# netneurolab/pypyls

Measured on AMD Instinct MI355X. Metric: resamples/sec (perm+boot), behavioral_pls X(500x200000)/Y(500x50) fp64, higher is better.
Workload: dtype f64

## Files before the change

### pypyls_amd/csrc/plsx_compact.hip

```cpp
#include "plsx_internal.h"

using namespace plsxi;

namespace plsxi {

template <int MT, int KT, bool TAIL = false>
int launch_xprod_cboot(plsx_ctx* ctx, int nres, int nks_c, SplitEpi se, hipStream_t st)
{
    se.nmu = compact_moment_rows(ctx) ? ctx->Tp : 0;
    const size_t lds = compact_lds_bytes(MT, KT, 3, nks_c, se.npairs);
    HIPCHK(set_lds(k_xprod_compact<MT, KT, 3, TAIL>, lds));
    const int ncolblk = ceil_div(ctx->Bpad, 128);
    KTimer tm(ctx, KC_XPROD, st);
    hipLaunchKernelGGL((k_xprod_compact<MT, KT, 3, TAIL>), dim3(round_up(ncolblk, 8) * round_up(nres, 8)), dim3(256),
                       lds, st, ptr<double>(ctx->Afrag_c), (size_t)nks_c * MT * 64, ptr<double>(ctx->Xc), ctx->Bpad, nks_c,
                       ptr<double>(ctx->R), ctx->Bpad, ctx->Tpp, ptr<int>(ctx->out_row_c), ptr<int>(ctx->mom_idx_c),
                       ptr<double>(ctx->momn_m), nres, ncolblk, se);
    LAUNCHCHK();
    return 0;
}

int launch_cboot(plsx_ctx* ctx, int nres, int nks_c, SplitEpi se, hipStream_t st)
{
    const int MTc = ceil_div(ctx->Tp, 16);
    const bool tail = ctx->Tp - (MTc - 1) * 16 <= 4 && MTc >= 2;
    switch (MTc) {
        case 1: return launch_xprod_cboot<1, 12>(ctx, nres, nks_c, se, st);
        case 2: return tail ? launch_xprod_cboot<2, 6, true>(ctx, nres, nks_c, se, st)
                            : launch_xprod_cboot<2, 6>(ctx, nres, nks_c, se, st);
        case 3: return tail ? launch_xprod_cboot<3, 4, true>(ctx, nres, nks_c, se, st)
                            : launch_xprod_cboot<3, 4>(ctx, nres, nks_c, se, st);
        case 4: return tail ? launch_xprod_cboot<4, PLSX_CKT, true>(ctx, nres, nks_c, se, st)
                            : launch_xprod_cboot<4, PLSX_CKT>(ctx, nres, nks_c, se, st);
#define PLSX_CB(M, K) case M: return tail ? launch_xprod_cboot<M, K, true>(ctx, nres, nks_c, se, st) \
                                          : launch_xprod_cboot<M, K>(ctx, nres, nks_c, se, st);
        PLSX_CB(5, 2) PLSX_CB(6, 2) PLSX_CB(7, 1) PLSX_CB(8, 1) PLSX_CB(9, 1) PLSX_CB(10, 1) PLSX_CB(11, 1) PLSX_CB(12, 1) PLSX_CB(13, 1)
#undef PLSX_CB
        default: return fail(ctx, PLSX_ERR_STATE, "compact bootstrap blocks: T' > 208");
    }
}
template <int MT, int KT, bool TAIL = false, int EPI = 5>
int launch_xprod_compact(plsx_ctx* ctx, int m, int nks_c, SplitEpi se, hipStream_t st)
{
    const int J = ctx->J;
    const size_t lds = compact_lds_bytes(MT, KT, EPI, nks_c, J);
    se.off_pre = 0;
    HIPCHK(set_lds(k_xprod_compact<MT, KT, EPI, TAIL>, lds));
    const int ncolblk = ceil_div(ctx->Bpad, 128);
    KTimer tm(ctx, KC_XPROD, st);
    hipLaunchKernelGGL((k_xprod_compact<MT, KT, EPI, TAIL>), dim3(round_up(ncolblk, 8) * round_up(m, 8)), dim3(256), lds, st,
                       ptr<double>(ctx->Afrag_c), (size_t)nks_c * MT * 64, ptr<double>(ctx->Xc), ctx->Bpad, nks_c,
                       ptr<double>(ctx->R), ctx->Bpad, (EPI == 8 ? 1 : 2) * ctx->Tpp, ptr<int>(ctx->out_row_c), ptr<int>(ctx->mom_idx_c),
                       ptr<double>(ctx->momn_m), m, ncolblk, se);
    LAUNCHCHK();
    return 0;
}

int launch_csplit(plsx_ctx* ctx, int m, int nks_c, SplitEpi se, hipStream_t st, bool raw)
// ... 28 lines not shown
```

### pypyls_amd/csrc/plsx_core.hip

```cpp
#include "plsx_internal.h"
#include "plsx_resample.h"
using namespace plsxi;

namespace plsxi {

const char* const kKernelClassNames[KC_COUNT] = {"k_xprod", "k_gram", "k_small", "k_urot", "k_nt_gemm",
                                                 "k_ucorr_partial", "k_simpls_dual", "k_build_A", "k_xprod_moments",
                                                 "k_sd_cv_score", "k_sd_coef", "k_coef_prod", "k_percentile", "k_contrast", "k_mb_rownorm",
                                                 "k_sd_cv_class"};

int plan_groups(plsx_ctx* c)
{
    const bool mb = c->method == PLSX_MULTIBLOCK;
    c->scaled = ((c->method == PLSX_BEHAVIORAL || mb) && !c->cov) ? 1 : 0;
    c->momrows = ((c->method == PLSX_BEHAVIORAL && (!c->cov || c->cv_mom)) || (mb && !c->cov)) ? 1 : 0;
    const int Jw = c->momrows ? c->J : 0;
    c->gps = 0;
    c->h_slice_row0.clear(); c->h_slice_rows.clear(); c->h_slice_cell0.clear(); c->h_slice_ncell.clear();
    auto fit = [&](int mt) {
        int b = 0;
        for (int n = 1; n <= 512; ++n) {
            int td = ceil_div(n * c->Tp, 16), tw = Jw ? ceil_div(n * Jw, 16) : 0;
            if (td + 2 * tw <= mt && tw * 16 <= 48) b = n; else break;
        }
// ... 1231 lines not shown
    ctx->timing = enable ? 1 : 0;
    for (auto& ev : ctx->events) { (void)hipEventDestroy(ev.e0); (void)hipEventDestroy(ev.e1); }
    ctx->events.clear();
    ctx->timed_units = 0;
    ctx->nt_flops = 0.0;
    ctx->quad_series = 0;
    return PLSX_OK;
} PLSX_CATCH(ctx)

int plsx_last_timing(const plsx_ctx* cctx, double* out, int cap)
try {
    plsx_ctx* ctx = const_cast<plsx_ctx*>(cctx);
    if (!ctx || !out || cap < 1) return PLSX_ERR_ARG;
    double ms = 0.0;
    int launches = 0;
    for (auto& ev : ctx->events) {
        if (ev.cls != KC_XPROD) continue;
        float t = 0.f;
        if (hipEventSynchronize(ev.e1) == hipSuccess && hipEventElapsedTime(&t, ev.e0, ev.e1) == hipSuccess)
            ms += t;
        ++launches;
    }
    double crows = 0.0;
    if (ctx->last_compact_n > 0) {
        std::vector<int> cnt(ctx->last_compact_n);
        if (hipMemcpy(cnt.data(), ptr<int>(ctx->rowtab_c) + (size_t)ctx->last_compact_n * ctx->last_compact_ktot,
                      cnt.size() * sizeof(int), hipMemcpyDeviceToHost) == hipSuccess) {
            for (int c : cnt) crows += 4.0 * ((std::max(c, 1) + 3) / 4);
            crows /= (double)cnt.size() * ctx->S;
        }
    }
    const bool cmp = ctx->last_compact_n > 0;
    const auto uvar = [&](int nks) { return (double)(nks > 0 && ctx->urot_tail_l ? nks + 100 : nks); };
    double vals[23] = {ms, (double)launches, (double)(cmp ? 1 : (ctx->sepmom_used ? ctx->npg_d : ctx->npg)),
                       (double)(cmp ? ceil_div(ctx->Tp, 16) : (ctx->sepmom_used ? ctx->MTd : ctx->MT)),
                       (double)ctx->Gcap * ctx->npg, (double)ctx->timed_units, (double)use_dual(ctx), crows,
                       ctx->nt_flops, (double)ctx->quad_series, (double)ctx->quad_MT, (double)ctx->quad_gpl,
                       (double)ctx->urot_waves_l, (double)ctx->urot_splits_l, (double)ctx->urot_rps_l,
                       uvar(ctx->urot_nks_first), (double)ctx->gram_chunks_l, uvar(ctx->urot_nks_last),
                       (double)ctx->gram_kind_l, (double)ctx->split_blocks_l, (double)ctx->split_reader_l,
                       (double)(cmp && ctx->last_moment_rows ? 1 : 0), (double)ctx->last_perm_projected};
    int n = std::min(cap, 23);
    for (int i = 0; i < n; ++i) out[i] = vals[i];
    return n;
} PLSX_CATCH(const_cast<plsx_ctx*>(cctx))

int plsx_kernel_timing(const plsx_ctx* cctx, int kernel_class, double* ms_out, int* launches_out)
try {
    plsx_ctx* ctx = const_cast<plsx_ctx*>(cctx);
    if (!ctx || kernel_class < 0 || kernel_class >= KC_COUNT) return PLSX_ERR_ARG;
    double ms = 0.0;
    int launches = 0;
    for (auto& ev : ctx->events) {
        if (ev.cls != kernel_class) continue;
        float t = 0.f;
        if (hipEventSynchronize(ev.e1) == hipSuccess && hipEventElapsedTime(&t, ev.e0, ev.e1) == hipSuccess)
            ms += t;
        ++launches;
    }
    if (ms_out) *ms_out = ms;
    if (launches_out) *launches_out = launches;
    return PLSX_OK;
} PLSX_CATCH(const_cast<plsx_ctx*>(cctx))

const char* plsx_kernel_class_name(int kernel_class)
{
    return (kernel_class >= 0 && kernel_class < KC_COUNT) ? kKernelClassNames[kernel_class] : nullptr;
}

int plsx_set_perm_path(plsx_ctx* ctx, int dual)
try {
    NEED_DATA();
    if (dual >= 0) ctx->dual = (dual && ctx->dual_ok) ? 1 : 0;
    ctx->has_Kd = 0;
    return use_dual(ctx);
// ... 136 lines not shown
```

### pypyls_amd/csrc/plsx_internal.h

```cpp
#pragma once
#include "plsx_kernels.h"
#include <chrono>
#include "../../include/plsx.h"

#include <algorithm>
#include <cmath>
#include <cstdio>
#include <cstdlib>
#include <cstring>
#include <new>
#include <stdexcept>
#include <string>
#include <thread>
#include <vector>

struct Buf {
    void* p = nullptr;
    size_t bytes = 0;
};

enum {
    OPT_NO_REFINE = 0, OPT_MIN_BATCH, OPT_INBLOCK_MOMENTS, OPT_NO_COMPACT_BOOT, OPT_COMPACT_BOOT_ALWAYS,
    OPT_SEPMOM_ALWAYS, OPT_NO_GRAM4, OPT_UROT_GENERIC, OPT_UROT_NO_TAIL4, OPT_NO_FIXED_X, OPT_NO_DUAL_PERM,
    OPT_TWO_PASS_BOOT, OPT_SPLIT_INBLOCK, OPT_NO_SPLIT_FUSE, OPT_SPLIT_TWO_READERS, OPT_EXPECT_RESAMPLES,
    OPT_SIMPLS_JACOBI, OPT_PERCENTILE_SORT, OPT_QUAD_SUMS, OPT_SPLIT_READER8, OPT_SIMPLS_GLOBAL,
    OPT_CROSSCOV_SPARSE, OPT_NO_MOMENT_ROWS, OPT_NO_PERM_PROJECT, OPT_COUNT
};
static const char* const kOptionNames[OPT_COUNT] = {
    "no_refine", "min_batch", "inblock_moments", "no_compact_boot", "compact_boot_always",
    "sepmom_always", "no_gram4", "urot_generic", "urot_no_tail4", "no_fixed_x", "no_dual_perm",
    "two_pass_boot", "split_inblock", "no_split_fuse", "split_two_readers", "expect_resamples",
    "simpls_jacobi", "percentile_sort", "quad_sums", "split_reader8", "simpls_global",
    "crosscov_sparse", "no_moment_rows", "no_perm_project"};

#ifndef PLSX_CKT
#define PLSX_CKT 3
#endif

struct plsx_ctx {
    int device = 0;
    std::string err;
    int opt[OPT_COUNT] = {};
    bool has_data = false, has_orig = false;
    int method = 0, S = 0, B = 0, T = 0, J = 0, n_groups = 0, n_cond = 1, mc = 0, cov = 0;
    int Tp = 0, Tpp = 0, L = 0, Kpad = 0, nks = 0, Bx = 0, Bpad = 0;
    int MT = 24, npg = 0, w0 = 0, sq0 = 0, nmom_pad = 0, scaled = 0, momrows = 0, Gcap = 0, Galloc = 0;
    int nks_t = 0, LT = 0, cv_mom = 0;
    int afrag_group0 = 0;
    int sepmom = 0, MTd = 0, npg_d = 0, sepmom_used = 0;
    size_t group_stride_d = 0;
    Buf out_row_d, mom_idx_d, Afrag_m, momn_m, scale;
    Buf Afrag_c, rank_c, rowtab_c, m1_c, m2_c, out_row_c, mom_idx_c, mask_c;
    int has_compact_maps = 0;
    size_t group_stride = 0;
    int gps = 0;
    Buf row_slice, row_local, slice_cell0, cell_momrow;
    std::vector<int> h_slice_row0, h_slice_rows, h_slice_cell0, h_slice_ncell;
    int fix = 0, has_Xn = 0, MTf = 25, npgf = 0;
    size_t group_stride_f = 0;
    long long strideR = 0;
    std::vector<int> h_cell_start, h_cell_len;
    Buf Xc, xmean, Y, cell_of_row, cell_start, cell_len, out_row, mom_idx, mom_n;
    Buf Afrag, R, Gm, Pm, part, Mfrag, U0T, V0, d0, tmpW;
    Buf Rfull, Vp, dp, Mvd, Cm, srcx, srcy, part2;
    Buf Kmat, swork, spct, sc;
    Buf momout, R2, cvc, Qm, Vs, ds, ybar, pred;
    Buf Xn, out_row_f, mom_idx_f;
    Buf Kd, Ad, Wd;
    Buf Zcv;
// ... 28 lines not shown
    int quad_active = 0;
    long long quad_n = 0, series_total = 0;
    Buf Cc, Asumc, Adc, Qc;
    int coef_active = 0, coef_c = 0;
    long long coef_n = 0;
    double* keepA = nullptr;
    long long keep_cap = 0, keep_n = 0;
    Buf cichunk;
    double* vipG = nullptr;
    long long vip_cap = 0, vip_n = 0;
    int vip_c = 0;
    int cperm_active = 0, cperm_c = 0, cperm_std = 0;
    const double* cperm_obs = nullptr;
    int* cperm_count = nullptr;
    double* cperm_max = nullptr;
    long long cperm_cap = 0, cperm_n = 0;
    Buf cpA, cppart, colsd;
    Buf cls, clsfreq;
    int has_cls = 0, cls_active = 0;
    int* cls_conf = nullptr;
    long long cls_cap = 0, cls_n = 0;
    bool has_okx = false, has_oky = false;
    int n_okx = 0;
    double* mom_out_arg = nullptr;
    int ncomp = 0;
    int timing = 0;
    struct TimedEv { int cls; hipEvent_t e0, e1; };
    std::vector<TimedEv> events;
    long long timed_units = 0;
    double nt_flops = 0.0;
    int quad_MT = 0, quad_gpl = 0, quad_series = 0;
    int last_compact_n = 0, last_compact_ktot = 0;
    int last_moment_rows = 0;
    int urot_waves_l = 0, urot_splits_l = 0, urot_rps_l = 0;
    int urot_nks_first = 0, urot_nks_last = 0, urot_tail_l = 0;
    int gram_chunks_l = 0, gram_kind_l = 0;
    double scratch_gb = 48.0;
    long long R_geom[6] = {0, 0, 0, 0, 0, 0};
    size_t R_zeroed_bytes = 0;
    double map_ms_per_gb = 0.0;
    int scratch_fixed = 0;
    double last_ms = 0.0;
    int last_launches = 0;
    void* comm = nullptr;
    int comm_rank = 0, comm_world = 1;
    int comm_team = 0;
};

namespace plsxi {


inline int fail(plsx_ctx* c, int code, const std::string& msg)
{
    if (c) c->err = msg;
    return code;
}

inline int fail_nothrow(plsx_ctx* c, int code, const char* what) noexcept
{
    if (c) {
        try { c->err = what ? what : "exception"; } catch (...) { }
    }
    return code;
}
#define PLSX_CATCH(ctxexpr)                                                                            \
    catch (const std::bad_alloc&) { return fail_nothrow(ctxexpr, PLSX_ERR_HIP, "out of host memory"); } \
// ... 113 lines not shown
int note_spectrum(plsx_ctx* ctx, const double* d_sv, hipStream_t st, int* all_live = nullptr);
struct QuadSet { Buf* C; Buf* Vsum; const double* Vd; int L; };
int quad_accumulate(plsx_ctx* ctx, int m, hipStream_t st, const QuadSet* qs = nullptr);
bool quad_applicable(const plsx_ctx* ctx);
int run_contrast_norms(plsx_ctx* ctx, int nres, double* out_sv, hipStream_t st);
int run_contrast_fill(plsx_ctx* ctx, int nres, hipStream_t st);
int run_percentile(plsx_ctx* ctx, const double* d_data, long long nseries, int n, int i_lo, double g_lo, int i_hi,
                   double g_hi, double* d_lo, double* d_hi, hipStream_t st);
inline void coef_close(plsx_ctx* ctx)
{
    ctx->coef_active = 0; ctx->coef_n = 0;
    ctx->keepA = nullptr; ctx->keep_cap = 0; ctx->keep_n = 0;
}
inline void vip_close(plsx_ctx* ctx)
{
    ctx->vipG = nullptr; ctx->vip_cap = 0; ctx->vip_n = 0; ctx->vip_c = 0;
}
inline void cperm_close(plsx_ctx* ctx)
{
    ctx->cperm_active = 0; ctx->cperm_c = 0; ctx->cperm_std = 0;
    ctx->cperm_obs = nullptr; ctx->cperm_count = nullptr; ctx->cperm_max = nullptr;
    ctx->cperm_cap = 0; ctx->cperm_n = 0;
}
inline void cls_close(plsx_ctx* ctx)
{
    ctx->cls_active = 0; ctx->cls_conf = nullptr; ctx->cls_cap = 0; ctx->cls_n = 0;
}
int launch_xprod(plsx_ctx* ctx, int groups, hipStream_t st);
int launch_xprod_acc(plsx_ctx* ctx, const double* Afrag, size_t gstride, int groups, int L, hipStream_t st);
int run_xprod_fixed(plsx_ctx* ctx, const int* ysrc, int nres, hipStream_t st, const double* ystack);
int run_xprod_fixed_norms(plsx_ctx* ctx, const int* ysrc, int nres, hipStream_t st, const double* ystack, double* out_sv);
MomLayout moment_layout(const plsx_ctx* ctx, int npairs);
MomLayout moment2_layout(const plsx_ctx* ctx, int npairs);
int compact_boot_ksteps(int mt);
bool compact_moment_rows(const plsx_ctx* ctx);
int launch_moment_blocks_raw(plsx_ctx* ctx, const MomLayout& ml, SplitEpi se, hipStream_t st);
int ensure_compact_maps(plsx_ctx* ctx);
int run_mb_rownorm(plsx_ctx* ctx, int nres, hipStream_t st);
int run_xprod(plsx_ctx* ctx, const int* xsrc, const int* ysrc, int nres, hipStream_t st,
              bool prebuilt = false, const double* ystack = nullptr, long long ystride = -1, bool sparse_rows = false);
int launch_xprod_split(plsx_ctx* ctx, int groups, SplitEpi se, hipStream_t st);
int quad_finish(plsx_ctx* ctx, double* d_usum, double* d_usq, hipStream_t st, const QuadSet* qs = nullptr);
inline int quad_blocks(int tiles) { return tiles >= 8 ? ceil_div(tiles, 8) : 1; }
int launch_cboot(plsx_ctx* ctx, int nres, int nks_c, SplitEpi se, hipStream_t st);
int launch_csplit(plsx_ctx* ctx, int m, int nks_c, SplitEpi se, hipStream_t st, bool raw = false);
int run_nt(plsx_ctx* ctx, const double* A, long long strideA, int lda, int Ma,
           const double* B1, long long strideB1, int ldb1, int N1,
           const double* B2, long long strideB2, int ldb2, int N2, int K, int batch,
           double* C1, long long strideC1, int ldc1, double* C2, long long strideC2, int ldc2,
           hipStream_t st, bool sym = false, bool accumulate = false, bool one_chunk = false);
bool nt_sym_fits(int S);
int nt_strips(plsx_ctx* ctx, const double* A, int lda, int Ma, const double* Bm, int ldb, int N, int Kc,
              double* C, int ldc, hipStream_t st, bool one_chunk = false);
int form_gram_K(plsx_ctx* ctx, const double* X, int ldx, int S, int Kc, double* K, int ldk, hipStream_t st);
int run_dual_gp(plsx_ctx* ctx, int m, int Sd, const double* ScT, int L, hipStream_t st);
int run_gram_ex(plsx_ctx* ctx, int nres, int mode, const double* E, int Erows, double* Pout,
                hipStream_t st, const double* Rsrc = nullptr);
int run_gram(plsx_ctx* ctx, int nres, bool with_p, hipStream_t st);
int run_small(plsx_ctx* ctx, SmallArgs a, int nres, hipStream_t st, const double* Rref = nullptr);
int launch_small_ql(plsx_ctx* ctx, const SmallArgs& a, int nres, size_t ws, size_t lds, hipStream_t st);
int launch_small_ql_refined(plsx_ctx* ctx, const SmallArgs& a, int nres, size_t ws, size_t lds, hipStream_t st);
int run_urot(plsx_ctx* ctx, int nres, double* usum, double* usq, double* out, hipStream_t st);
int launch_ucorr(plsx_ctx* ctx, dim3 grid, dim3 block, hipStream_t st, const double* M, int tpc,
                 double* part, int npairs);
int ucorr_slots();
bool simpls_single_pass(const plsx_ctx* ctx);
size_t simpls_global_lds_bytes(int T, int k);
// ... 5 lines not shown
```

### pypyls_amd/csrc/plsx_k_xprod.h

```cpp
#pragma once
#include <type_traits>
#include <utility>

template <class F, int... I>
__device__ __forceinline__ void xprod_static_for(F&& f, std::integer_sequence<int, I...>)
{
    (f(std::integral_constant<int, I>()), ...);
}
#include "plsx_common.h"
#include "plsx_k_prep.h"

#define PLSX_RSRC_FLAGS 0x00020000
template <int NT, int PASSES, bool EVEN, int STAGE>
__device__ __forceinline__ void stage_copy_buf(const double* src, double* dst, int tid, int wave)
{
    __amdgpu_buffer_rsrc_t rs = __builtin_amdgcn_make_buffer_rsrc((void*)src, (short)0, 0x7fffffff,
                                                                   PLSX_RSRC_FLAGS);
    const int voff = tid * 16;
#pragma unroll
    for (int p = 0; p < PASSES; ++p) {
        if (EVEN || p * NT + wave * 64 < STAGE / 2) {
            __builtin_amdgcn_raw_ptr_buffer_load_lds(
                rs, (__attribute__((address_space(3))) void*)(dst + (size_t)(p * NT + wave * 64) * 2),
                16, voff, p * NT * 16, 0, 0);
// ... 383 lines not shown
                double* mo = mom_out + ((size_t)grp * nmom_pad + mr) * 2 * ldr + col;
                mo[0] = m1 / nn;
                mo[ldr] = sc;
            }
        }
        __syncthreads();
    }
    if (NW > 4 && col >= ldr) return;
    double* Rg = R + (size_t)(ntab > 1 ? grp / ntab : grp) * rows_per_group * ldr + col;
#pragma unroll
    for (int m = 0; m < W0; ++m) {
        int orow[4];
        double sc[4];
#pragma unroll
        for (int i = 0; i < 4; ++i) {
            const int row = m * 16 + kq + 4 * i;
            orow[i] = s_out[row];
            const int mi = s_mom[row];
            sc[i] = (NSQ > 0 && mi >= 0) ? sS[mi * 16 + (lane & 15)] : 1.0;
        }
#pragma unroll
        for (int i = 0; i < 4; ++i)
            if (orow[i] >= 0) Rg[(size_t)orow[i] * ldr] = acc[m][i] * sc[i];
    }
}

__device__ __forceinline__ d2 load_x2_buf(const double* base, int voff)
{
    __amdgpu_buffer_rsrc_t rs = __builtin_amdgcn_make_buffer_rsrc((void*)base, (short)0, 0x7fffffff, PLSX_RSRC_FLAGS);
    return __builtin_bit_cast(d2, __builtin_amdgcn_raw_buffer_load_b128(rs, voff, 0, 0));
}

__host__ __device__ constexpr int compact_stage_lds(int MT, int KT) { return ((KT * MT * 64 + 127) / 128) * 128; }
__host__ __device__ constexpr int compact_scale_regs(int KT) { return KT < 4 ? KT : 4; }
__host__ __device__ constexpr size_t compact_lds_bytes(int MT, int KT, int EPI, int nks, int J)
{
    const size_t loop = (size_t)MT * 16 * 8 + (size_t)2 * compact_stage_lds(MT, KT) * 8 + (size_t)nks * 4 * 4;
    if (EPI == 3) return loop + (J > compact_scale_regs(KT) ? (size_t)J * 128 * 8 : 0);
    const size_t epi5 = (size_t)MT * 16 * 8 + (size_t)5 * J * 128 * 8 + (size_t)MT * 16 * 5 * 8;
    return EPI == 5 && epi5 > loop ? epi5 : loop;
}

__host__ __device__ constexpr int compact_waves(int MT, int EPI, bool TAIL)
{
    if (EPI == 3 && MT == 2) return TAIL ? 7 : 6;
    if (EPI == 3) return MT > 10 ? 2 : MT == 10 ? (TAIL ? 3 : 2) : MT > 6 ? 3 : MT > 4 ? 4 : (MT == 4 && TAIL) ? 5 : 4;
    return (EPI == 5 && MT == 4 && !TAIL) ? 3 : 4;
}

template <int MT, int KT, int EPI, bool TAIL>
__global__ __launch_bounds__(256, compact_waves(MT, EPI, TAIL))
void k_xprod_compact(const double* __restrict__ Afrag, size_t group_stride,
                     const double* __restrict__ X, int ldx, int nks,
                     double* __restrict__ R, int ldr, int rows_per_group,
                     const int* __restrict__ out_row, const int* __restrict__ mom_idx,
                     const double* __restrict__ mom_n, int n_groups, int ncolblk, SplitEpi se)
{
    static_assert(EPI == 3 || EPI == 5 || EPI == 8, "compact blocks: bootstrap (3), fused split-half (5) or raw first-half sums (8)");
    extern __shared__ __attribute__((aligned(16))) double smem[];
    constexpr int NW = 4, NT = NW * 64, BC = NW * 32;
    constexpr int STAGE = KT * MT * 64;
    constexpr int STAGE_LDS = compact_stage_lds(MT, KT);
    constexpr int PASSES = (STAGE + NT * 2 - 1) / (NT * 2);
    constexpr bool EVEN = (STAGE % (NT * 2)) == 0;
    constexpr int MF = TAIL ? MT - 1 : MT;
    constexpr int NSCR = compact_scale_regs(KT);
    static_assert(MT * 16 <= NT, "the row maps are staged by one thread per row");
    const int ncb = (ncolblk + 7) & ~7;
    const int sweep = blockIdx.x / (8 * ncb);
    const int within = blockIdx.x - sweep * (8 * ncb);
    const int slot = within >> 3;
    const int grp = sweep * 8 + (slot & 7);
    const int colblk = (slot >> 3) * 8 + (within & 7);
    if (grp >= n_groups || colblk >= ncolblk) return;
    const double* Ag = Afrag + (size_t)grp * group_stride;
    const int swave = __builtin_amdgcn_readfirstlane((int)threadIdx.x >> 6);

    d4 acc0[MF > 0 ? MF : 1], acc1[MF > 0 ? MF : 1];
#pragma unroll
    for (int m = 0; m < MF; ++m) { acc0[m] = (d4){0.0, 0.0, 0.0, 0.0}; acc1[m] = (d4){0.0, 0.0, 0.0, 0.0}; }
    double tl0 = 0.0, tl1 = 0.0;

    int* s_out = reinterpret_cast<int*>(smem);
    int* s_mom = s_out + MT * 16;
    double* sStage = smem + MT * 16;
    int* s_tab = reinterpret_cast<int*>(sStage + 2 * STAGE_LDS);
    const int J3 = se.npairs;
    double* sW = reinterpret_cast<double*>(s_tab + nks * 4) + swave * (J3 * 32);
    d2 scr[NSCR];
    const int mrow0 = (EPI == 3) ? se.nmu : 0;
    int cnt_lo[NSCR], cnt_hi[NSCR];
    {
// ... 295 lines not shown
```

### pypyls_amd/csrc/plsx_xprod.hip

```cpp
#include "plsx_internal.h"

using namespace plsxi;

namespace plsxi {

template <int MT, int NW, int KT, int NSQ>
int launch_xprod_t(plsx_ctx* ctx, int groups, hipStream_t st)
{
    const size_t stage = (size_t)2 * (((size_t)KT * MT * 64 + 127) / 128) * 128 * 8;
    const size_t epi = (size_t)NW * 2 * NSQ * 16 * 16 * 8 + (size_t)2 * MT * 16 * 4;
    const size_t lds = std::max(stage, epi);
    HIPCHK(set_lds(k_xprod<MT, NW, KT, NSQ>, lds));
    const int ncolblk = ctx->Bpad / (NW * 16);
    dim3 grid(ncolblk * round_up(groups, 8)), block(NW * 64);
    KTimer tm(ctx, KC_XPROD, st);
    hipLaunchKernelGGL((k_xprod<MT, NW, KT, NSQ>), grid, block, lds, st,
                       ptr<double>(ctx->Afrag) + (size_t)ctx->afrag_group0 * ctx->group_stride, ctx->group_stride,
                       ptr<double>(ctx->Xc), ctx->Bpad,
                       ctx->nks, ptr<double>(ctx->R), ctx->Bpad, ctx->npg * ctx->Tpp,
                       ptr<int>(ctx->out_row), ptr<int>(ctx->mom_idx), ptr<double>(ctx->mom_n),
                       std::max(ctx->nmom_pad, 0), groups, ncolblk, ctx->mom_out_arg,
                       SplitEpi{nullptr, nullptr, nullptr, nullptr, nullptr, 0, 0}, std::max(ctx->gps, 1));
    LAUNCHCHK();
    return 0;
// ... 270 lines not shown
int ensure_compact_maps(plsx_ctx* ctx)
{
    if (ctx->has_compact_maps) return 0;
    const int rows = ceil_div(ctx->Tp, 16) * 16;
    std::vector<int> orow(rows, -1), mrow(rows, -1);
    for (int t = 0; t < ctx->Tp; ++t) { orow[t] = t; mrow[t] = t / ctx->T; }
    if (int e = ensure(ctx, ctx->out_row_c, rows * sizeof(int))) return e;
    if (int e = ensure(ctx, ctx->mom_idx_c, rows * sizeof(int))) return e;
    HIPCHK(hipMemcpy(ctx->out_row_c.p, orow.data(), rows * sizeof(int), hipMemcpyHostToDevice));
    HIPCHK(hipMemcpy(ctx->mom_idx_c.p, mrow.data(), rows * sizeof(int), hipMemcpyHostToDevice));
    ctx->has_compact_maps = 1;
    return 0;
}

int launch_moment_blocks_raw(plsx_ctx* ctx, const MomLayout& ml, SplitEpi se, hipStream_t st)
{
    return launch_moment_blocks<6>(ctx, ml, se, st);
}

bool compact_boot_ok(const plsx_ctx* ctx)
{
    if (!(ctx->scaled && ctx->method == PLSX_BEHAVIORAL && ctx->gps == 0 && ctx->Tp <= 208 && !ctx->mom_out_arg &&
          ctx->J <= 32 && ctx->S <= 8192 && (long long)ctx->Kpad * ctx->Bpad * 8 < (1LL << 31)))
        return false;
    const int force = ctx->opt[OPT_COMPACT_BOOT_ALWAYS] ? 1 : (ctx->opt[OPT_NO_COMPACT_BOOT] ? -1 : 0);
    if (force) return force > 0;
    const int mt = ceil_div(ctx->Tp, 16);
    const double rows = (mt >= 2 && ctx->Tp - (mt - 1) * 16 <= 4) ? (mt - 1) * 16 + 4 : mt * 16;
    const double cost_c = 0.66 * 1.25 * rows / 16.0;
    const int npg_dense = ctx->sepmom ? ctx->npg_d : ctx->npg, mt_dense = ctx->sepmom ? ctx->MTd : ctx->MT;
    return cost_c * 1.1 < (double)mt_dense / npg_dense && npg_dense <= 16;
}

int compact_boot_ksteps(int mt) { return mt == 4 ? PLSX_CKT : std::max(1, 12 / mt); }

bool compact_moment_rows(const plsx_ctx* ctx)
{
    if (ctx->opt[OPT_NO_MOMENT_ROWS]) return false;
    const int mt = ceil_div(ctx->Tp, 16);
    const bool tail = mt >= 2 && ctx->Tp - (mt - 1) * 16 <= 4;
    const int rows = tail ? (mt - 1) * 16 + 4 : mt * 16;
    return ctx->J <= compact_scale_regs(compact_boot_ksteps(mt)) && rows - ctx->Tp >= ctx->J;
}

int run_xprod_cboot(plsx_ctx* ctx, const int* xsrc, const int* ysrc, int nres, hipStream_t st,
                    const double* ystack, long long ystride)
{
    const int S = ctx->S, J = ctx->J, MTc = ceil_div(ctx->Tp, 16), KT = compact_boot_ksteps(MTc);
    const int nks_c = round_up(ceil_div(S, 4), KT);
    const int npairs = nres * J;
    const bool mrows = compact_moment_rows(ctx);
    const MomLayout ml = mrows ? moment2_layout(ctx, npairs) : moment_layout(ctx, npairs);
    const int groups_m = ml.groups;
    const size_t astride = (size_t)nks_c * MTc * 64, mstride = ml.stride;
    if (int e = ensure_compact_maps(ctx)) return e;
    if (int e = ensure(ctx, ctx->Afrag_c, (size_t)nres * astride * 8 + 4096)) return e;
    if (int e = ensure(ctx, ctx->mask_c, (size_t)nres * S)) return e;
    if (int e = ensure(ctx, ctx->rank_c, (size_t)nres * S * sizeof(int))) return e;
    if (int e = ensure(ctx, ctx->rowtab_c, ((size_t)nres * nks_c * 4 + nres) * sizeof(int))) return e;
    if (int e = ensure(ctx, ctx->Afrag_m, (size_t)groups_m * mstride * 8 + 4096)) return e;
    if (int e = ensure(ctx, ctx->momn_m, (size_t)round_up(npairs, 384) * 8)) return e;
    if (int e = ensure(ctx, ctx->scale, (size_t)round_up(npairs, 8) * ctx->Bpad * 8)) return e;
    HIPCHK(hipMemsetAsync(ctx->Afrag_c.p, 0, (size_t)nres * astride * 8, st));
    HIPCHK(hipMemsetAsync(ctx->Afrag_m.p, 0, (size_t)groups_m * mstride * 8, st));
    HIPCHK(hipMemsetAsync(ctx->mask_c.p, 0, (size_t)nres * S, st));
    int* row_cnt = ptr<int>(ctx->rowtab_c) + (size_t)nres * nks_c * 4;
    ctx->last_compact_n = nres; ctx->last_compact_ktot = nks_c * 4; ctx->last_moment_rows = mrows ? 1 : 0;
    {
        KTimer tm(ctx, KC_BUILD, st);
        hipLaunchKernelGGL(k_drawn_mask, dim3(ceil_div(S, 256), nres), dim3(256), 0, st, xsrc, S, ptr<uint8_t>(ctx->mask_c));
        LAUNCHCHK();
        hipLaunchKernelGGL(k_split_rank, dim3(nres), dim3(64), 0, st, ptr<uint8_t>(ctx->mask_c), S, nks_c * 4,
                           ptr<int>(ctx->rank_c), ptr<int>(ctx->rowtab_c), row_cnt);
        LAUNCHCHK();
        GroupLayout lay;
        lay.n = 1; lay.Tp = ctx->Tp; lay.J = J; lay.T = ctx->T; lay.MT = MTc; lay.w0 = MTc; lay.sq0 = MTc; lay.Tpp = ctx->Tpp;
        int cap = 0;
        const size_t blds = build_lds_behav(ctx, &cap);
        hipLaunchKernelGGL(k_build_A_behav, dim3(nres, J), dim3(256), blds, st,
                           ystack ? ystack : ptr<double>(ctx->Y), ystack ? ystride : 0LL, ctx->T, S,
                           ptr<int>(ctx->cell_start), ptr<int>(ctx->cell_len), xsrc, ysrc, lay, ctx->cov, 1,
                           ptr<double>(ctx->Afrag_c), astride, ptr<double>(ctx->momn_m), 0, 0,
                           ptr<double>(ctx->Afrag_m), mstride, ptr<int>(ctx->rank_c), ml.pairs, cap, mrows ? ctx->Tp : -1);
        LAUNCHCHK();
    }
    SplitEpi se;
    memset(&se, 0, sizeof(se));
    se.scale = ptr<double>(ctx->scale);
    se.npairs = npairs;
    if (int e = mrows ? launch_moment_blocks<9>(ctx, ml, se, st) : launch_moment_blocks<4>(ctx, ml, se, st)) return e;
    se.npairs = J;
    se.accB = nres * ctx->Tpp;
    se.row_tab = ptr<int>(ctx->rowtab_c);
    se.row_cnt = row_cnt;
    return launch_cboot(ctx, nres, nks_c, se, st);
}

int run_mb_rownorm(plsx_ctx* ctx, int nres, hipStream_t st)
{
    const int cols = mb_chunk_cols(ctx->B), nchunk = ceil_div(ctx->B, cols);
// ... 178 lines not shown
```

### pypyls_amd/engine.py

```python
import ctypes
import threading
import os

import numpy as np

from . import _build

_LIB = None

PLSX_BEHAVIORAL = 0
PLSX_MEANCENTERED = 1
PLSX_REGRESSION = 2
PLSX_FLAG_COVARIANCE = 1


class PlsxError(RuntimeError):
    pass


def _load():
    global _LIB
    if _LIB is not None:
        return _LIB
    import torch
# ... 841 lines not shown
        self.sync()
        shp = boot.shape[:-1]
        return lo.cpu().numpy().reshape(shp), hi.cpu().numpy().reshape(shp)

    def mfma_f64_peak(self):
        v = ctypes.c_double()
        self._check(self.lib.plsx_mfma_f64_peak(self.ctx, ctypes.byref(v)))
        return v.value

    def set_timing(self, enable=True):
        self._check(self.lib.plsx_set_timing(self.ctx, 1 if enable else 0))

    def kernel_timing(self):
        out = {}
        k = 0
        while True:
            name = self.lib.plsx_kernel_class_name(k)
            if not name:
                break
            ms, n = ctypes.c_double(), ctypes.c_int()
            self._check(self.lib.plsx_kernel_timing(self.ctx, k, ctypes.byref(ms), ctypes.byref(n)))
            if n.value:
                out[name.decode()] = (ms.value, n.value)
            k += 1
        return out

    def set_perm_path(self, dual):
        rc = self.lib.plsx_set_perm_path(self.ctx, -1 if dual is None else (1 if dual else 0))
        if rc < 0:
            self._check(rc)
        return bool(rc)

    def last_timing(self):
        buf = (ctypes.c_double * 23)()
        n = self.lib.plsx_last_timing(self.ctx, buf, 23)
        keys = ['xprod_ms', 'xprod_launches', 'resamples_per_group', 'm_tiles', 'superbatch',
                'xprod_resamples', 'dual_perm', 'compact_row_fraction', 'nt_flops', 'quad_series', 'quad_m_tiles',
                'quad_blocks_per_lv', 'urot_waves', 'urot_splits', 'urot_res_per_split', 'urot_variant',
                'gram_chunks', 'urot_variant_last', 'gram_kernel', 'split_blocks', 'split_reader',
                'moment_rows', 'perm_projected']
        return {k: buf[i] for i, k in enumerate(keys[:max(n, 0)])}


_DEFAULT = {}
_DEFAULT_LOCK = threading.Lock()


def default_engine(device=None, replica=0):
    torch = _torch()
    if device is None:
        device = torch.cuda.current_device() if torch.cuda.is_available() else 0
    key = (int(device), int(replica))
    with _DEFAULT_LOCK:
        eng = _DEFAULT.get(key)
        if eng is None or not getattr(eng, 'ctx', None):
            if not _DEFAULT:
                import atexit
                atexit.register(release_default_engine)
            eng = _DEFAULT[key] = Engine(device=key[0])
    return eng


IDLE_RELEASE_S = 300.0
_IDLE = {'timer': None}


def touch_idle_release():
    if not IDLE_RELEASE_S:
        return
    with _DEFAULT_LOCK:
        old = _IDLE['timer']
        if old is not None:
            old.cancel()
# ... 37 lines not shown
```

Baseline: 6256.

## Add four-column-tile compact bootstrap kernel variant for tail-shaped T'

Result: faster. 6354 (median of 6 runs) (+1.6%).

```diff
diff --git a/pypyls_amd/csrc/plsx_compact.hip b/pypyls_amd/csrc/plsx_compact.hip
--- a/pypyls_amd/csrc/plsx_compact.hip
+++ b/pypyls_amd/csrc/plsx_compact.hip
@@ -4,15 +4,15 @@
 
 namespace plsxi {
 
-template <int MT, int KT, bool TAIL = false>
+template <int MT, int KT, bool TAIL = false, int NC = 2>
 int launch_xprod_cboot(plsx_ctx* ctx, int nres, int nks_c, SplitEpi se, hipStream_t st)
 {
     se.nmu = compact_moment_rows(ctx) ? ctx->Tp : 0;
-    const size_t lds = compact_lds_bytes(MT, KT, 3, nks_c, se.npairs);
-    HIPCHK(set_lds(k_xprod_compact<MT, KT, 3, TAIL>, lds));
-    const int ncolblk = ceil_div(ctx->Bpad, 128);
+    const size_t lds = compact_lds_bytes(MT, KT, 3, nks_c, se.npairs, NC);
+    HIPCHK(set_lds(k_xprod_compact<MT, KT, 3, TAIL, NC>, lds));
+    const int ncolblk = ceil_div(ctx->Bpad, 64 * NC);
     KTimer tm(ctx, KC_XPROD, st);
-    hipLaunchKernelGGL((k_xprod_compact<MT, KT, 3, TAIL>), dim3(round_up(ncolblk, 8) * round_up(nres, 8)), dim3(256),
+    hipLaunchKernelGGL((k_xprod_compact<MT, KT, 3, TAIL, NC>), dim3(round_up(ncolblk, 8) * round_up(nres, 8)), dim3(256),
                        lds, st, ptr<double>(ctx->Afrag_c), (size_t)nks_c * MT * 64, ptr<double>(ctx->Xc), ctx->Bpad, nks_c,
                        ptr<double>(ctx->R), ctx->Bpad, ctx->Tpp, ptr<int>(ctx->out_row_c), ptr<int>(ctx->mom_idx_c),
                        ptr<double>(ctx->momn_m), nres, ncolblk, se);
@@ -24,6 +24,18 @@
 {
     const int MTc = ceil_div(ctx->Tp, 16);
     const bool tail = ctx->Tp - (MTc - 1) * 16 <= 4 && MTc >= 2;
+    if (compact_boot_wide(ctx)) {
+        switch (MTc) {
+            case 1: return launch_xprod_cboot<1, 6, false, 4>(ctx, nres, nks_c, se, st);
+            case 2: return tail ? launch_xprod_cboot<2, 4, true, 4>(ctx, nres, nks_c, se, st)
+                                : launch_xprod_cboot<2, 4, false, 4>(ctx, nres, nks_c, se, st);
+            case 3: return tail ? launch_xprod_cboot<3, 3, true, 4>(ctx, nres, nks_c, se, st)
+                                : launch_xprod_cboot<3, 3, false, 4>(ctx, nres, nks_c, se, st);
+            case 4: return tail ? launch_xprod_cboot<4, PLSX_CKTW, true, 4>(ctx, nres, nks_c, se, st)
+                                : launch_xprod_cboot<4, PLSX_CKTW, false, 4>(ctx, nres, nks_c, se, st);
+            default: return fail(ctx, PLSX_ERR_STATE, "compact bootstrap blocks of 256 columns: T' > 64");
+        }
+    }
     switch (MTc) {
         case 1: return launch_xprod_cboot<1, 12>(ctx, nres, nks_c, se, st);
         case 2: return tail ? launch_xprod_cboot<2, 6, true>(ctx, nres, nks_c, se, st)
diff --git a/pypyls_amd/csrc/plsx_core.hip b/pypyls_amd/csrc/plsx_core.hip
--- a/pypyls_amd/csrc/plsx_core.hip
+++ b/pypyls_amd/csrc/plsx_core.hip
@@ -1287,15 +1287,16 @@
     }
     const bool cmp = ctx->last_compact_n > 0;
     const auto uvar = [&](int nks) { return (double)(nks > 0 && ctx->urot_tail_l ? nks + 100 : nks); };
-    double vals[23] = {ms, (double)launches, (double)(cmp ? 1 : (ctx->sepmom_used ? ctx->npg_d : ctx->npg)),
+    double vals[24] = {ms, (double)launches, (double)(cmp ? 1 : (ctx->sepmom_used ? ctx->npg_d : ctx->npg)),
                        (double)(cmp ? ceil_div(ctx->Tp, 16) : (ctx->sepmom_used ? ctx->MTd : ctx->MT)),
                        (double)ctx->Gcap * ctx->npg, (double)ctx->timed_units, (double)use_dual(ctx), crows,
                        ctx->nt_flops, (double)ctx->quad_series, (double)ctx->quad_MT, (double)ctx->quad_gpl,
                        (double)ctx->urot_waves_l, (double)ctx->urot_splits_l, (double)ctx->urot_rps_l,
                        uvar(ctx->urot_nks_first), (double)ctx->gram_chunks_l, uvar(ctx->urot_nks_last),
                        (double)ctx->gram_kind_l, (double)ctx->split_blocks_l, (double)ctx->split_reader_l,
-                       (double)(cmp && ctx->last_moment_rows ? 1 : 0), (double)ctx->last_perm_projected};
-    int n = std::min(cap, 23);
+                       (double)(cmp && ctx->last_moment_rows ? 1 : 0), (double)ctx->last_perm_projected,
+                       (double)(cmp ? (ctx->last_compact_wide ? 4 : 2) : 0)};
+    int n = std::min(cap, 24);
     for (int i = 0; i < n; ++i) out[i] = vals[i];
     return n;
 } PLSX_CATCH(const_cast<plsx_ctx*>(cctx))
diff --git a/pypyls_amd/csrc/plsx_internal.h b/pypyls_amd/csrc/plsx_internal.h
--- a/pypyls_amd/csrc/plsx_internal.h
+++ b/pypyls_amd/csrc/plsx_internal.h
@@ -24,17 +24,20 @@
     OPT_SEPMOM_ALWAYS, OPT_NO_GRAM4, OPT_UROT_GENERIC, OPT_UROT_NO_TAIL4, OPT_NO_FIXED_X, OPT_NO_DUAL_PERM,
     OPT_TWO_PASS_BOOT, OPT_SPLIT_INBLOCK, OPT_NO_SPLIT_FUSE, OPT_SPLIT_TWO_READERS, OPT_EXPECT_RESAMPLES,
     OPT_SIMPLS_JACOBI, OPT_PERCENTILE_SORT, OPT_QUAD_SUMS, OPT_SPLIT_READER8, OPT_SIMPLS_GLOBAL,
-    OPT_CROSSCOV_SPARSE, OPT_NO_MOMENT_ROWS, OPT_NO_PERM_PROJECT, OPT_COUNT
+    OPT_CROSSCOV_SPARSE, OPT_NO_MOMENT_ROWS, OPT_NO_PERM_PROJECT, OPT_NO_COMPACT_WIDE, OPT_COMPACT_WIDE_ALWAYS, OPT_COUNT
 };
 static const char* const kOptionNames[OPT_COUNT] = {
     "no_refine", "min_batch", "inblock_moments", "no_compact_boot", "compact_boot_always",
     "sepmom_always", "no_gram4", "urot_generic", "urot_no_tail4", "no_fixed_x", "no_dual_perm",
     "two_pass_boot", "split_inblock", "no_split_fuse", "split_two_readers", "expect_resamples",
     "simpls_jacobi", "percentile_sort", "quad_sums", "split_reader8", "simpls_global",
-    "crosscov_sparse", "no_moment_rows", "no_perm_project"};
+    "crosscov_sparse", "no_moment_rows", "no_perm_project", "no_compact_wide", "compact_wide_always"};
 
 #ifndef PLSX_CKT
 #define PLSX_CKT 3
+#endif
+#ifndef PLSX_CKTW
+#define PLSX_CKTW 2
 #endif
 
 struct plsx_ctx {
@@ -129,6 +132,7 @@
     int quad_MT = 0, quad_gpl = 0, quad_series = 0;
     int last_compact_n = 0, last_compact_ktot = 0;
     int last_moment_rows = 0;
+    int last_compact_wide = 0;
     int urot_waves_l = 0, urot_splits_l = 0, urot_rps_l = 0;
     int urot_nks_first = 0, urot_nks_last = 0, urot_tail_l = 0;
     int gram_chunks_l = 0, gram_kind_l = 0;
@@ -308,7 +312,8 @@
 int run_xprod_fixed_norms(plsx_ctx* ctx, const int* ysrc, int nres, hipStream_t st, const double* ystack, double* out_sv);
 MomLayout moment_layout(const plsx_ctx* ctx, int npairs);
 MomLayout moment2_layout(const plsx_ctx* ctx, int npairs);
-int compact_boot_ksteps(int mt);
+bool compact_boot_wide(const plsx_ctx* ctx);
+int compact_boot_ksteps(int mt, bool wide);
 bool compact_moment_rows(const plsx_ctx* ctx);
 int launch_moment_blocks_raw(plsx_ctx* ctx, const MomLayout& ml, SplitEpi se, hipStream_t st);
 int ensure_compact_maps(plsx_ctx* ctx);
diff --git a/pypyls_amd/csrc/plsx_k_xprod.h b/pypyls_amd/csrc/plsx_k_xprod.h
--- a/pypyls_amd/csrc/plsx_k_xprod.h
+++ b/pypyls_amd/csrc/plsx_k_xprod.h
@@ -439,24 +439,275 @@
 }
 
 __host__ __device__ constexpr int compact_stage_lds(int MT, int KT) { return ((KT * MT * 64 + 127) / 128) * 128; }
-__host__ __device__ constexpr int compact_scale_regs(int KT) { return KT < 4 ? KT : 4; }
-__host__ __device__ constexpr size_t compact_lds_bytes(int MT, int KT, int EPI, int nks, int J)
+__host__ __device__ constexpr int compact_scale_regs(int KT, int NC = 2) { return KT < 4 ? KT : 4; }
+__host__ __device__ constexpr size_t compact_lds_bytes(int MT, int KT, int EPI, int nks, int J, int NC = 2)
 {
     const size_t loop = (size_t)MT * 16 * 8 + (size_t)2 * compact_stage_lds(MT, KT) * 8 + (size_t)nks * 4 * 4;
-    if (EPI == 3) return loop + (J > compact_scale_regs(KT) ? (size_t)J * 128 * 8 : 0);
+    if (EPI == 3) return loop + (J > compact_scale_regs(KT, NC) ? (size_t)J * (64 * NC) * 8 : 0);
     const size_t epi5 = (size_t)MT * 16 * 8 + (size_t)5 * J * 128 * 8 + (size_t)MT * 16 * 5 * 8;
     return EPI == 5 && epi5 > loop ? epi5 : loop;
 }
 
-__host__ __device__ constexpr int compact_waves(int MT, int EPI, bool TAIL)
+__host__ __device__ constexpr int compact_waves(int MT, int EPI, bool TAIL, int NC = 2)
 {
+    if (NC == 4) return MT == 1 ? 4 : (MT == 4 && !TAIL) ? 2 : 3;
     if (EPI == 3 && MT == 2) return TAIL ? 7 : 6;
     if (EPI == 3) return MT > 10 ? 2 : MT == 10 ? (TAIL ? 3 : 2) : MT > 6 ? 3 : MT > 4 ? 4 : (MT == 4 && TAIL) ? 5 : 4;
     return (EPI == 5 && MT == 4 && !TAIL) ? 3 : 4;
 }
 
-template <int MT, int KT, int EPI, bool TAIL>
-__global__ __launch_bounds__(256, compact_waves(MT, EPI, TAIL))
+template <int MT, int KT, bool TAIL>
+__device__ __forceinline__ void compact_wide_block(double* smem, const double* __restrict__ Afrag, size_t group_stride,
+                                                   const double* __restrict__ X, int ldx, int nks,
+                                                   double* __restrict__ R, int ldr, int rows_per_group,
+                                                   const int* __restrict__ out_row, const int* __restrict__ mom_idx,
+                                                   const double* __restrict__ mom_n, int n_groups, int ncolblk,
+                                                   const SplitEpi& se)
+{
+    constexpr int NC = 4, NW = 4, NT = NW * 64, BC = NW * 16 * NC;
+    constexpr int STAGE = KT * MT * 64;
+    constexpr int STAGE_LDS = compact_stage_lds(MT, KT);
+    constexpr int PASSES = (STAGE + NT * 2 - 1) / (NT * 2);
+    constexpr bool EVEN = (STAGE % (NT * 2)) == 0;
+    constexpr int MF = TAIL ? MT - 1 : MT;
+    constexpr int NSCR = compact_scale_regs(KT, NC);
+    static_assert(MT * 16 <= NT, "the row maps are staged by one thread per row");
+    const int ncb = (ncolblk + 7) & ~7;
+    const int sweep = blockIdx.x / (8 * ncb);
+    const int within = blockIdx.x - sweep * (8 * ncb);
+    const int slot = within >> 3;
+    const int grp = sweep * 8 + (slot & 7);
+    const int colblk = (slot >> 3) * 8 + (within & 7);
+    if (grp >= n_groups || colblk >= ncolblk) return;
+    const double* Ag = Afrag + (size_t)grp * group_stride;
+    const int swave = __builtin_amdgcn_readfirstlane((int)threadIdx.x >> 6);
+
+    d4 acc[NC][MF > 0 ? MF : 1];
+    double tl[NC];
+#pragma unroll
+    for (int c = 0; c < NC; ++c) {
+        tl[c] = 0.0;
+#pragma unroll
+        for (int m = 0; m < MF; ++m) acc[c][m] = (d4){0.0, 0.0, 0.0, 0.0};
+    }
+
+    int* s_out = reinterpret_cast<int*>(smem);
+    double* sStage = smem + MT * 16;
+    int* s_tab = reinterpret_cast<int*>(sStage + 2 * STAGE_LDS);
+    const int J3 = se.npairs;
+    double* sW = reinterpret_cast<double*>(s_tab + nks * 4) + swave * (J3 * 64);
+    d2 scr[NSCR][2];
+    const int mrow0 = se.nmu;
+    int cnt_lo[NSCR], cnt_hi[NSCR];
+    {
+    const int tid = threadIdx.x, lane = tid & 63, wave = tid >> 6;
+    const int kq = lane >> 4;
+    const int cw = wave * 64 + 4 * (lane & 15);
+    const int col = colblk * BC + cw;
+    const bool live = col < ldr;
+    const int lcol8 = (live ? col : 0) * 8;
+    const int toff = (lane & 48) + (lane & 3) - lane;
+
+    const int* tabg = se.row_tab + (size_t)grp * nks * 4;
+    const int ldx8 = ldx * 8;
+    int row0[KT];
+#pragma unroll
+    for (int s = 0; s < KT; ++s) row0[s] = tabg[s * 4 + kq];
+    stage_copy_buf<NT, PASSES, EVEN, STAGE>(Ag, sStage, tid, swave);
+    int orw = -1, mix = -1;
+    if (tid < MT * 16) {
+        orw = out_row[tid];
+        mix = mom_idx[tid];
+    }
+    const int ksteps = max(1, (se.row_cnt[grp] + 3) >> 2);
+    const int nkt = (ksteps + KT - 1) / KT;
+    const int ntab = nkt * KT * 4;
+    auto tab_load = [&](int i0, int (&v)[4]) {
+#pragma unroll
+        for (int u = 0; u < 4; ++u) v[u] = tabg[min(i0 + u * NT + tid, ntab - 1)];
+#pragma unroll
+        for (int u = 0; u < 4; ++u) asm volatile("" : "+v"(v[u]));
+    };
+    auto tab_store = [&](int i0, const int (&v)[4]) {
+#pragma unroll
+        for (int u = 0; u < 4; ++u)
+            if (i0 + u * NT + tid < ntab) s_tab[i0 + u * NT + tid] = v[u] * ldx8;
+    };
+    int tv[4];
+    tab_load(0, tv);
+    d2 xa[KT][2], xb[KT][2];
+#pragma unroll
+    for (int s = 0; s < KT; ++s) {
+        xa[s][0] = load_x2_buf(X, row0[s] * ldx8 + lcol8);
+        xa[s][1] = load_x2_buf(X, row0[s] * ldx8 + lcol8 + 16);
+    }
+    tab_store(0, tv);
+    for (int i0 = 4 * NT; i0 < ntab; i0 += 4 * NT) { tab_load(i0, tv); tab_store(i0, tv); }
+    if (tid < MT * 16) {
+        const int rows_valid = min(rows_per_group, se.accB - grp * rows_per_group);
+        s_out[tid] = (orw < 0 || orw >= rows_valid) ? -1 : (orw | ((mix + 1) << 16));
+    }
+#pragma unroll
+    for (int s = 0; s < KT; ++s) { asm volatile("" : "+v"(xa[s][0])); asm volatile("" : "+v"(xa[s][1])); }
+    __syncthreads();
+
+    const double* sA0 = sStage + lane;
+    const double* sT0 = sA0 + toff;
+    auto contract = [&](auto curc, const d2 (&xc)[KT][2], auto full, int nlive) {
+        const int cur = curc;
+        const double* sA = sA0 + cur * STAGE_LDS;
+        const double* sT = sT0 + cur * STAGE_LDS;
+#pragma unroll
+        for (int s = 0; s < KT; ++s) {
+            if (!decltype(full)::value && s >= nlive) continue;
+            const double b[NC] = {xc[s][0].x, xc[s][0].y, xc[s][1].x, xc[s][1].y};
+#pragma unroll
+            for (int m = 0; m < MF; ++m) {
+                const double a = sA[(s * MT + m) * 64];
+#pragma unroll
+                for (int c = 0; c < NC; ++c) acc[c][m] = mfma_f64(a, b[c], acc[c][m]);
+            }
+            if constexpr (TAIL) {
+                const double a = sT[(s * MT + MT - 1) * 64];
+#pragma unroll
+                for (int c = 0; c < NC; ++c) tl[c] = mfma_f64_4x4(a, b[c], tl[c]);
+            }
+        }
+    };
+    const int* tp = s_tab + KT * 4 + kq;
+    const double* An = Ag + STAGE;
+    auto pass = [&](auto curc, const d2 (&xc)[KT][2], d2 (&xn)[KT][2]) {
+        constexpr int CUR = decltype(curc)::value;
+        stage_copy_buf<NT, PASSES, EVEN, STAGE>(An, sStage + (CUR ^ 1) * STAGE_LDS, tid, swave);
+#pragma unroll
+        for (int s = 0; s < KT; ++s) {
+            xn[s][0] = load_x2_buf(X, tp[s * 4] + lcol8);
+            xn[s][1] = load_x2_buf(X, tp[s * 4] + lcol8 + 16);
+        }
+        An += STAGE;
+        tp += KT * 4;
+        contract(curc, xc, std::true_type(), KT);
+        __syncthreads();
+    };
+    auto last = [&](int cur, const d2 (&xc)[KT][2]) {
+#pragma unroll
+        for (int j = 0; j < NSCR; ++j) { scr[j][0] = scr[j][1] = (d2){1.0, 1.0}; cnt_lo[j] = 0; cnt_hi[j] = 0; }
+        if (J3 <= NSCR) {
+            if (mrow0 > 0) {
+#pragma unroll
+                for (int j = 0; j < NSCR; ++j)
+                    if (j < J3) {
+                        const double v = mom_n[(size_t)grp * J3 + j];
+                        cnt_lo[j] = __builtin_amdgcn_readfirstlane(__double2loint(v));
+                        cnt_hi[j] = __builtin_amdgcn_readfirstlane(__double2hiint(v));
+                    }
+            }
+#pragma unroll
+            for (int j = 0; j < NSCR; ++j)
+                if (j < J3) {
+                    const char* p = reinterpret_cast<const char*>(se.scale + ((size_t)grp * J3 + j) * ldr) + lcol8;
+                    scr[j][0] = *reinterpret_cast<const d2*>(p);
+                    scr[j][1] = *reinterpret_cast<const d2*>(p + 16);
+                }
+        } else if (live) {
+            __amdgpu_buffer_rsrc_t rs = __builtin_amdgcn_make_buffer_rsrc(
+                (void*)(se.scale + (size_t)grp * J3 * ldr + colblk * BC + swave * 64), (short)0, 0x7fffffff, PLSX_RSRC_FLAGS);
+            const int ln4 = __lane_id() * 4;
+            for (int j = 0; j < J3; ++j) {
+                __builtin_amdgcn_raw_ptr_buffer_load_lds(
+                    rs, (__attribute__((address_space(3))) void*)(sW + j * 64), 4, ln4, j * ldr * 8, 0, 0);
+                __builtin_amdgcn_raw_ptr_buffer_load_lds(
+                    rs, (__attribute__((address_space(3))) void*)(sW + j * 64 + 32), 4, ln4, j * ldr * 8 + 256, 0, 0);
+            }
+        }
+        contract(cur, xc, std::false_type(), ksteps - (nkt - 1) * KT);
+    };
+    {
+        std::integral_constant<int, 0> c0;
+        std::integral_constant<int, 1> c1;
+        int kt = 0, cur = 0;
+        for (; kt + 2 < nkt; kt += 2) { pass(c0, xa, xb); pass(c1, xb, xa); }
+        if (kt + 1 < nkt) {
+            pass(c0, xa, xb);
+#pragma unroll
+            for (int s = 0; s < KT; ++s) { xa[s][0] = xb[s][0]; xa[s][1] = xb[s][1]; }
+            cur = 1;
+        }
+        last(cur, xa);
+    }
+    }
+
+    if (mrow0 > 0 && J3 <= NSCR) {
+        const int ln = __lane_id();
+        const int q = ln >> 4;
+#pragma unroll
+        for (int j = 0; j < NSCR; ++j) {
+            if (j >= J3) continue;
+            const int r = mrow0 + j;
+            const int src = ((r & 3) << 4) | (ln & 15);
+            double m1 = 0.0;
+#pragma unroll
+            for (int c = 0; c < NC; ++c) {
+                double a;
+                if constexpr (TAIL) a = tl[c];
+                else {
+                    const int ri = (r & 15) >> 2;
+                    a = acc[c][MT - 1][0];
+#pragma unroll
+                    for (int i = 1; i < 4; ++i)
+                        if (ri == i) a = acc[c][MT - 1][i];
+                }
+                const double v = __shfl(a, src);
+                if (q == c) m1 = v;
+            }
+            const double nn = __hiloint2double(cnt_hi[j], cnt_lo[j]);
+            const double m2 = q == 0 ? scr[j][0].x : q == 1 ? scr[j][0].y : q == 2 ? scr[j][1].x : scr[j][1].y;
+            const double var = (m2 - m1 * m1 / nn) / (nn - 1.0);
+            double sc = (var > 0.0) ? sd_rsqrt(var) : 0.0;
+            asm volatile("" : "+v"(sc));
+            const int c15 = ln & 15;
+            scr[j][0] = (d2){__shfl(sc, c15), __shfl(sc, c15 | 16)};
+            scr[j][1] = (d2){__shfl(sc, c15 | 32), __shfl(sc, c15 | 48)};
+        }
+    }
+
+    int tid16 = threadIdx.x * 16;
+    asm volatile("" : "+v"(tid16));
+    const int tid = tid16 >> 4, lane = tid & 63, wave = tid >> 6, kq = lane >> 4;
+    const int cw = wave * 64 + 4 * (lane & 15), col = colblk * BC + cw;
+    if (col >= ldr) return;
+    if (J3 > NSCR) asm volatile("s_waitcnt vmcnt(0)" ::: "memory");
+    double* Rg = R + (size_t)grp * rows_per_group * ldr + col;
+#pragma unroll
+    for (int m = 0; m < MT; ++m)
+#pragma unroll
+        for (int i = 0; i < 4; ++i) {
+            if (TAIL && m == MT - 1 && i > 0) break;
+            const int packed = s_out[m * 16 + kq + 4 * i];
+            if (packed < 0) continue;
+            const int orow = packed & 0xffff, mi = (packed >> 16) - 1;
+            d2 s0 = (d2){1.0, 1.0}, s1 = (d2){1.0, 1.0};
+            if (J3 > NSCR) {
+                if (mi >= 0) {
+                    s0 = *reinterpret_cast<const d2*>(&sW[mi * 64 + 4 * (lane & 15)]);
+                    s1 = *reinterpret_cast<const d2*>(&sW[mi * 64 + 4 * (lane & 15) + 2]);
+                }
+            } else {
+#pragma unroll
+                for (int j = 0; j < NSCR; ++j)
+                    if (mi == j) { s0 = scr[j][0]; s1 = scr[j][1]; }
+            }
+            double v[NC];
+#pragma unroll
+            for (int c = 0; c < NC; ++c) v[c] = (TAIL && m == MT - 1) ? tl[c] : acc[c][m < MF ? m : 0][i];
+            d2* dst = reinterpret_cast<d2*>(&Rg[(size_t)orow * ldr]);
+            dst[0] = (d2){v[0] * s0.x, v[1] * s0.y};
+            dst[1] = (d2){v[2] * s1.x, v[3] * s1.y};
+        }
+}
+
+template <int MT, int KT, int EPI, bool TAIL, int NC = 2>
+__global__ __launch_bounds__(256, compact_waves(MT, EPI, TAIL, NC))
 void k_xprod_compact(const double* __restrict__ Afrag, size_t group_stride,
                      const double* __restrict__ X, int ldx, int nks,
                      double* __restrict__ R, int ldr, int rows_per_group,
@@ -464,7 +715,13 @@
                      const double* __restrict__ mom_n, int n_groups, int ncolblk, SplitEpi se)
 {
     static_assert(EPI == 3 || EPI == 5 || EPI == 8, "compact blocks: bootstrap (3), fused split-half (5) or raw first-half sums (8)");
+    static_assert(NC == 2 || (NC == 4 && EPI == 3 && MT <= 4), "four column tiles per wave: bootstraps of up to four tiles");
     extern __shared__ __attribute__((aligned(16))) double smem[];
+    if constexpr (NC == 4) {
+        compact_wide_block<MT, KT, TAIL>(smem, Afrag, group_stride, X, ldx, nks, R, ldr, rows_per_group, out_row, mom_idx,
+                                         mom_n, n_groups, ncolblk, se);
+        return;
+    }
     constexpr int NW = 4, NT = NW * 64, BC = NW * 32;
     constexpr int STAGE = KT * MT * 64;
     constexpr int STAGE_LDS = compact_stage_lds(MT, KT);
diff --git a/pypyls_amd/csrc/plsx_xprod.hip b/pypyls_amd/csrc/plsx_xprod.hip
--- a/pypyls_amd/csrc/plsx_xprod.hip
+++ b/pypyls_amd/csrc/plsx_xprod.hip
@@ -326,7 +326,19 @@
     return cost_c * 1.1 < (double)mt_dense / npg_dense && npg_dense <= 16;
 }
 
-int compact_boot_ksteps(int mt) { return mt == 4 ? PLSX_CKT : std::max(1, 12 / mt); }
+bool compact_boot_wide(const plsx_ctx* ctx)
+{
+    const int mt = ceil_div(ctx->Tp, 16);
+    if (mt > 4 || ctx->opt[OPT_NO_COMPACT_WIDE]) return false;
+    if (ctx->opt[OPT_COMPACT_WIDE_ALWAYS]) return true;
+    return mt == 4 && ctx->Tp - (mt - 1) * 16 <= 4;
+}
+
+int compact_boot_ksteps(int mt, bool wide)
+{
+    if (wide) return mt == 4 ? PLSX_CKTW : mt == 3 ? 3 : mt == 2 ? 4 : 6;
+    return mt == 4 ? PLSX_CKT : std::max(1, 12 / mt);
+}
 
 bool compact_moment_rows(const plsx_ctx* ctx)
 {
@@ -334,13 +346,15 @@
     const int mt = ceil_div(ctx->Tp, 16);
     const bool tail = mt >= 2 && ctx->Tp - (mt - 1) * 16 <= 4;
     const int rows = tail ? (mt - 1) * 16 + 4 : mt * 16;
-    return ctx->J <= compact_scale_regs(compact_boot_ksteps(mt)) && rows - ctx->Tp >= ctx->J;
+    const bool wide = compact_boot_wide(ctx);
+    return ctx->J <= compact_scale_regs(compact_boot_ksteps(mt, wide), wide ? 4 : 2) && rows - ctx->Tp >= ctx->J;
 }
 
 int run_xprod_cboot(plsx_ctx* ctx, const int* xsrc, const int* ysrc, int nres, hipStream_t st,
                     const double* ystack, long long ystride)
 {
-    const int S = ctx->S, J = ctx->J, MTc = ceil_div(ctx->Tp, 16), KT = compact_boot_ksteps(MTc);
+    const bool wide = compact_boot_wide(ctx);
+    const int S = ctx->S, J = ctx->J, MTc = ceil_div(ctx->Tp, 16), KT = compact_boot_ksteps(MTc, wide);
     const int nks_c = round_up(ceil_div(S, 4), KT);
     const int npairs = nres * J;
     const bool mrows = compact_moment_rows(ctx);
@@ -360,6 +374,7 @@
     HIPCHK(hipMemsetAsync(ctx->mask_c.p, 0, (size_t)nres * S, st));
     int* row_cnt = ptr<int>(ctx->rowtab_c) + (size_t)nres * nks_c * 4;
     ctx->last_compact_n = nres; ctx->last_compact_ktot = nks_c * 4; ctx->last_moment_rows = mrows ? 1 : 0;
+    ctx->last_compact_wide = wide ? 1 : 0;
     {
         KTimer tm(ctx, KC_BUILD, st);
         hipLaunchKernelGGL(k_drawn_mask, dim3(ceil_div(S, 256), nres), dim3(256), 0, st, xsrc, S, ptr<uint8_t>(ctx->mask_c));
diff --git a/pypyls_amd/engine.py b/pypyls_amd/engine.py
--- a/pypyls_amd/engine.py
+++ b/pypyls_amd/engine.py
@@ -897,13 +897,13 @@
         return bool(rc)
 
     def last_timing(self):
-        buf = (ctypes.c_double * 23)()
-        n = self.lib.plsx_last_timing(self.ctx, buf, 23)
+        buf = (ctypes.c_double * 24)()
+        n = self.lib.plsx_last_timing(self.ctx, buf, 24)
         keys = ['xprod_ms', 'xprod_launches', 'resamples_per_group', 'm_tiles', 'superbatch',
                 'xprod_resamples', 'dual_perm', 'compact_row_fraction', 'nt_flops', 'quad_series', 'quad_m_tiles',
                 'quad_blocks_per_lv', 'urot_waves', 'urot_splits', 'urot_res_per_split', 'urot_variant',
                 'gram_chunks', 'urot_variant_last', 'gram_kernel', 'split_blocks', 'split_reader',
-                'moment_rows', 'perm_projected']
+                'moment_rows', 'perm_projected', 'compact_col_tiles']
         return {k: buf[i] for i, k in enumerate(keys[:max(n, 0)])}
 
 
```
